# JvanKatwijk/sdr-j-fm

Measured on AMD Instinct MI355X. Metric: IQ MSamples/s demodulated to 48 kHz stereo, higher is better.
Workload: dtype f32 (stage A: 3-term split-f16 MFMA with a per-tile block exponent, f32 accumulate); 1 GPU; config4; population=established, channels_per_gpu=4096, channels_total=4096, streams_per_gpu=4096, block_samples_per_channel=230400, parallelism=channels sharded, 1 rank/GPU

## Files before the change

### sdr-j-fm_amd/csrc/fmx_audio.hip

```cpp
#include "fmx_internal.h"
#include "fmx_fftconv.h"
#include <cstdlib>

namespace fmx {

typedef float v2f __attribute__((ext_vector_type(2)));

__global__ __launch_bounds__(64) void pcm_tail_kernel(DeviceBuffers B, CallGeom G, int channels) {
    const int ch = blockIdx.x * 64 + threadIdx.x + G.ch0;
    if (ch >= G.ch0 + channels) return;
    ChanState *st = &B.state[ch];
    const int frames = (int)(G.M1 - G.M0);
    const int cnt0 = st->pk_cnt;
    float L = st->pk_l, R = st->pk_r;
    int ev = st->pk_events;
    const int tiles = B.peaks_on ? (frames + C_TILE - 1) / C_TILE : 0;
    for (int tile = 0; tile < tiles; tile++) {
        const int i0 = tile * C_TILE, nfr = min(C_TILE, frames - i0);
        const float4 p = B.pk_part[(size_t)ch * B.pk_tiles + tile];
        const int w_first = (cnt0 + i0) / PK_WIN;
        const int to_end = (w_first + 1) * PK_WIN - (cnt0 + i0);
        L = fmaxf(L, p.x); R = fmaxf(R, p.y);
        if (to_end <= nfr) {
            B.pk_ring[(size_t)ch * PK_RING + (ev & (PK_RING - 1))] = make_float2(L, R);
            ev++;
            L = p.z; R = p.w;
        }
    }
    st->pk_l = L; st->pk_r = R; st->pk_events = ev; st->pk_cnt = (cnt0 + frames) % PK_WIN;
    if (B.params[ch].test_tone) st->tt_pos = (int)(((int64_t)st->tt_pos + frames) % TT_CYCLE);
}

constexpr int AF_HIST = (C_MAX_TAPS + 3) / 4 - 1;
constexpr int AF_VALID = 7 * C_TILE;
static_assert(AF_HIST + AF_VALID <= fftc::N, "block + history fit one transform");
static_assert(AUDIO_DELAY % 4 == 0, "the four phases of a frame are one aligned group of four ring entries");
#ifndef AF_WAVES_PER_SIMD
#define AF_WAVES_PER_SIMD 3
#endif
template <bool PEAKS>
__global__ __launch_bounds__(fftc::T, AF_WAVES_PER_SIMD) void audio_fft_kernel(DeviceTables T, DeviceBuffers B, CallGeom G, float2 *__restrict__ pcm) {
    __shared__ __attribute__((aligned(16))) float2 X[fftc::LDS_N];
    __shared__ int pkt[7][4];
    const int ch = blockIdx.y + G.ch0, t = threadIdx.x, lane = t & 63;
    const int64_t mb = G.M0 + (int64_t)blockIdx.x * AF_VALID;
    if (mb >= G.M1) return;
    const ChanParams P = B.params[ch];
    const AudioSet AS = T.audio_sets[P.audio_set];
    const float2 *__restrict__ dring = B.dring + (size_t)ch * (G.dring_mask + 1);
    const float2 *__restrict__ Gs = T.audio_spec + (size_t)P.audio_set * 4 * fftc::N;
    if (PEAKS && t < 28) pkt[t >> 2][t & 3] = 0;
    float2 acc[8];
#pragma unroll
    for (int q = 0; q < 8; q++) acc[q] = make_float2(0.f, 0.f);
    auto load_phase = [&](int p, float2 *a) {
#pragma unroll
        for (int k = 0; k < 8; k++) {
            const int64_t fr = mb - AF_HIST + t + fftc::T * k;
            const int64_t f0 = 4 * fr - AS.delay;
            a[k] = (f0 >= 0 && fr < G.M1) ? dring[(f0 + 3 - p) & G.dring_mask] : make_float2(0.f, 0.f);
        }
    };
    float2 a[8];
    load_phase(0, a);
#pragma unroll 1
    for (int p = 0; p < 4; p++) {
        __syncthreads();
        fftc::forward_slots(t, a, X, T.fft_w);
        fftc::times_spectrum(t, a, Gs + (size_t)p * fftc::N);
#pragma unroll
        for (int q = 0; q < 8; q++) { acc[q].x += a[q].x; acc[q].y += a[q].y; }
        if (p < 3) load_phase(p + 1, a);
    }
    __syncthreads();
    fftc::backward_slots(t, acc, X, T.fft_w);
    const float gl = P.volume * P.left_ch, gr = P.volume * P.right_ch;
    const ChanState *__restrict__ st = &B.state[ch];
    const int64_t F = st->fade_start_frame;
    const int Max = 24000;
    const int cnt0 = st->pk_cnt, tt0 = st->tt_pos;
#pragma unroll
    for (int k = 0; k < 8; k++) {
        const int rel = t + fftc::T * k - AF_HIST;
        const int64_t m = mb + rel;
        const bool live = rel >= 0 && rel < AF_VALID && m < G.M1;
        const int tile = rel >= 0 ? rel / C_TILE : 0;
        float al = acc[k].x * gl, ar = acc[k].y * gr;
        float pv[4] = {0.f, 0.f, 0.f, 0.f};
        if (live) {
            if (G.gain_fix && m - G.M0 < GAIN_FIX_FRAMES) {
                const float2 c = B.gfix[(size_t)ch * GAIN_FIX_FRAMES + (m - G.M0)];
                al += c.x; ar += c.y;
            }
            const int64_t since = m - F;
            if (since >= 0 && since < Max) {
                const float cnt = (float)(Max - (int)since);
                const float f = ((float)Max - cnt) / (float)Max;
                al *= f; ar *= f;
            }
            const int i = (int)(m - G.M0);
            if (P.test_tone) {
#pragma clang fp contract(off)
                const float level = 0.9f;
                al = al * (1.0f - level); ar = ar * (1.0f - level);
                const int pos = (int)(((int64_t)tt0 + i) % TT_CYCLE);
                if (pos >= TT_SILENT) {
                    const float smpl = level * B.tone[pos - TT_SILENT];
                    al = al + smpl; ar = ar + smpl;
                }
            }
            const int i_tile = (int)(mb - G.M0) + tile * C_TILE;
            const bool second = (cnt0 + i) / PK_WIN != (cnt0 + i_tile) / PK_WIN;
            if (PEAKS) { pv[second ? 2 : 0] = fabsf(al); pv[second ? 3 : 1] = fabsf(ar); }
            pcm[(size_t)ch * G.pcm_stride + (m - G.M0)] = make_float2(al, ar);
        }
        if (!PEAKS) {
        } else if (t < 192) {
#pragma unroll
            for (int q = 0; q < 4; q++) {
                int v = __float_as_int(pv[q]);
#define AF_MAX_STEP(ctrl, rmask) v = max(v, __builtin_amdgcn_update_dpp(0, v, ctrl, rmask, 0xf, false))
                AF_MAX_STEP(0x111, 0xf); AF_MAX_STEP(0x112, 0xf); AF_MAX_STEP(0x114, 0xf); AF_MAX_STEP(0x118, 0xf);
                AF_MAX_STEP(0x142, 0xa); AF_MAX_STEP(0x143, 0xc);
#undef AF_MAX_STEP
                if (lane == 63 && k >= 1) atomicMax(&pkt[k - 1][q], v);
            }
        } else if (live) {
#pragma unroll
            for (int q = 0; q < 4; q++) atomicMax(&pkt[tile][q], __float_as_int(pv[q]));
        }
    }
    if (!PEAKS) return;
    __syncthreads();
    const int tiles = (int)(((G.M1 - mb) < AF_VALID ? (G.M1 - mb) : AF_VALID) + C_TILE - 1) / C_TILE;
    if (t < tiles) B.pk_part[(size_t)ch * B.pk_tiles + 7 * blockIdx.x + t] = make_float4(__int_as_float(pkt[t][0]), __int_as_float(pkt[t][1]), __int_as_float(pkt[t][2]), __int_as_float(pkt[t][3]));
}


__global__ __launch_bounds__(GAIN_FIX_BACK) void gain_fix_kernel(DeviceTables T, DeviceBuffers B, CallGeom G, int channels) {
    __shared__ float2 A[GAIN_FIX_BACK];
    const int ch = blockIdx.x, t = threadIdx.x;
    const ChanParams &P = B.params[ch];
    ChanState *st = &B.state[ch];
    const float gl = P.volume * P.left_ch, gr = P.volume * P.right_ch;
    const bool valid = st->gain_valid != 0;
    const float dl = valid ? st->prev_gl - gl : 0.f, dr = valid ? st->prev_gr - gr : 0.f;
    float2 *out = B.gfix + (size_t)ch * GAIN_FIX_FRAMES;
    __syncthreads();
    if (t == 0) { st->prev_gl = gl; st->prev_gr = gr; st->gain_valid = 1; }
    if (dl == 0.f && dr == 0.f) { if (t < GAIN_FIX_FRAMES) out[t] = make_float2(0.f, 0.f); return; }
    const AudioSet AS = T.audio_sets[P.audio_set];
    const float2 *__restrict__ dring = B.dring + (size_t)ch * (G.dring_mask + 1);
    {
        const int q = t;
        float2 acc = make_float2(0.f, 0.f);
        if (q >= 1) {
            const int64_t j = G.J0 - q - AS.delay;
            if (AS.delay > 0) {
                const float *__restrict__ ha = T.audio_lp_taps + (size_t)P.audio_set * AUDIO_TAPS;
                for (int i = 0; i < AUDIO_TAPS; i++) {
                    const int64_t idx = j - i;
                    const float2 v = idx >= 0 ? dring[idx & G.dring_mask] : make_float2(0.f, 0.f);
                    acc.x = fmaf(ha[i], v.x, acc.x); acc.y = fmaf(ha[i], v.y, acc.y);
                }
            } else acc = j >= 0 ? dring[j & G.dring_mask] : make_float2(0.f, 0.f);
        }
        A[q] = acc;
    }
    __syncthreads();
    if (t < GAIN_FIX_FRAMES) {
        const int e = (int)(4 * (G.M0 + t) + 3 - G.J0);
        float2 c = make_float2(0.f, 0.f);
        for (int q = (e < -1 ? -e : 1); q < GAIN_FIX_BACK && e + q < RS_TAPS; q++) {
            const float h = T.rs_taps[e + q];
            c.x = fmaf(h, A[q].x, c.x); c.y = fmaf(h, A[q].y, c.y);
        }
        out[t] = make_float2(dl * c.x, dr * c.y);
    }
}

void launch_gain_fix(const DeviceTables &T, const DeviceBuffers &B, const CallGeom &G, int channels, hipStream_t s) {
    hipLaunchKernelGGL(gain_fix_kernel, dim3(channels), dim3(GAIN_FIX_BACK), 0, s, T, B, G, channels);
}

void launch_audio(const DeviceTables &T, const DeviceBuffers &B, const CallGeom &G, float2 *pcm,
                  int channels, hipStream_t s) {
    const int64_t frames = G.M1 - G.M0;
    if (frames <= 0) return;
    if (B.peaks_on) hipLaunchKernelGGL(audio_fft_kernel<true>, dim3((unsigned)((frames + AF_VALID - 1) / AF_VALID), channels), dim3(fftc::T), 0, s, T, B, G, pcm);
    else hipLaunchKernelGGL(audio_fft_kernel<false>, dim3((unsigned)((frames + AF_VALID - 1) / AF_VALID), channels), dim3(fftc::T), 0, s, T, B, G, pcm);
    hipLaunchKernelGGL(pcm_tail_kernel, dim3((channels + 63) / 64), dim3(64), 0, s, B, G, channels);
}

__global__ __launch_bounds__(256) void conv2_kernel(const float2 *__restrict__ x48, int64_t x_stride, const float *__restrict__ taps,
                                                    int p, int q, int nt, int64_t in0, int64_t out0, int64_t nout,
                                                    float2 *__restrict__ pcm, int64_t pcm_stride) {
    const int64_t i = (int64_t)blockIdx.x * 256 + threadIdx.x;
    if (i >= nout) return;
    const int ch = blockIdx.y;
    const int64_t mq = (out0 + i) * q, n0 = mq / p;
    const int ph = (int)(mq - n0 * p);
    const float *t = taps + (size_t)ph * nt;
    const float2 *x = x48 + (size_t)ch * x_stride + nt + (n0 - in0);
    float ar = 0.f, ai = 0.f;
    for (int k = 0; k < nt; k++) {
        if (n0 - k < 0) break;
        const float2 v = x[-k];
        ar = __fadd_rn(ar, __fmul_rn(t[k], v.x)); ai = __fadd_rn(ai, __fmul_rn(t[k], v.y));
    }
    pcm[(size_t)ch * pcm_stride + i] = make_float2(ar, ai);
}
__global__ __launch_bounds__(256) void conv2_shift_kernel(float2 *x48, int64_t x_stride, int nt, int64_t frames) {
    float2 *x = x48 + (size_t)blockIdx.x * x_stride;
    const int t = threadIdx.x;
    float2 v = make_float2(0.f, 0.f);
    if (t < nt) v = x[frames + t];
    __syncthreads();
    if (t < nt) x[t] = v;
}
void launch_conv2(float2 *x48, int64_t x_stride, const float *taps, int p, int q, int nt, int64_t in0, int64_t frames_in,
                  int64_t out0, int64_t nout, float2 *pcm, int64_t pcm_stride, int channels, hipStream_t s) {
    if (nout > 0)
        hipLaunchKernelGGL(conv2_kernel, dim3((unsigned)((nout + 255) / 256), channels), dim3(256), 0, s, x48, x_stride, taps, p, q, nt,
                           in0, out0, nout, pcm, pcm_stride);
    if (frames_in > 0) hipLaunchKernelGGL(conv2_shift_kernel, dim3(channels), dim3(256), 0, s, x48, x_stride, nt, frames_in);
}

}
```

Baseline: 286,600 MS/s.

## Load ring phase pairs as float4 and hoist FFT twiddles into registers

The audio FFT kernel now reads two polyphase ring entries per float4 load instead of one float2 per phase. When the whole window is in range it takes a fast path with no per-element bounds checks. The FFT twiddles for all three radix-8 stages are loaded once per block and kept in registers for the four forward passes and the backward pass. The spectrum coefficients are prefetched inside the forward FFT so their latency overlaps the LDS stages. The cost is higher register pressure (twiddles plus the float4 buffer), which could lower occupancy at the 3-waves-per-SIMD bound.

```diff
diff --git a/sdr-j-fm_amd/csrc/fmx_audio.hip b/sdr-j-fm_amd/csrc/fmx_audio.hip
--- a/sdr-j-fm_amd/csrc/fmx_audio.hip
+++ b/sdr-j-fm_amd/csrc/fmx_audio.hip
@@ -38,42 +38,110 @@
 #ifndef AF_WAVES_PER_SIMD
 #define AF_WAVES_PER_SIMD 3
 #endif
+__device__ __forceinline__ int af_tid() { int t = threadIdx.x; asm volatile("" : "+v"(t)); return t; }
+struct AfTwiddles { float2 w2048[7], w256[7], w32[7]; };
+__device__ __forceinline__ void af_forward(int t, float2 *a, float2 *X, const AfTwiddles &tw, float4 *hs, const float2 *__restrict__ Hs) {
+    using namespace fftc;
+    int base, j;
+    fwd8(a, tw.w2048); store_q<2048>(a, X, 0, t);
+    __syncthreads();
+    geom8<256>(t, base, j);
+    load_p<256>(a, X, base, j); fwd8(a, tw.w256); store_q<256>(a, X, base, j);
+    const float4 *H4 = reinterpret_cast<const float4 *>(Hs + 8 * t);
+#pragma unroll
+    for (int q = 0; q < 4; q++) hs[q] = H4[q];
+    __syncthreads();
+    geom8<32>(t, base, j);
+    load_p<32>(a, X, base, j); fwd8(a, tw.w32);
+#pragma unroll
+    for (int q = 0; q < 8; q++) {
+        float2 v = a[q];
+        v = quad_f1<-1>(j, v, quad_get<0x4E>(v));
+        a[q] = quad_f2(j, v, quad_get<0xB1>(v));
+    }
+}
+__device__ __forceinline__ void af_backward(int t, float2 *a, float2 *X, const AfTwiddles &tw) {
+    using namespace fftc;
+    int base, j;
+    geom8<32>(t, base, j);
+#pragma unroll
+    for (int q = 0; q < 8; q++) {
+        float2 v = a[q];
+        v = quad_b1<-1>(j, v, quad_get<0xB1>(v));
+        a[q] = quad_b2(j, v, quad_get<0x4E>(v));
+    }
+    inv8(a, tw.w32); store_p<32>(a, X, base, j);
+    __syncthreads();
+    geom8<256>(t, base, j);
+    load_q<256>(a, X, base, j); inv8(a, tw.w256); store_p<256>(a, X, base, j);
+    __syncthreads();
+    load_q<2048>(a, X, 0, t); inv8(a, tw.w2048);
+}
 template <bool PEAKS>
 __global__ __launch_bounds__(fftc::T, AF_WAVES_PER_SIMD) void audio_fft_kernel(DeviceTables T, DeviceBuffers B, CallGeom G, float2 *__restrict__ pcm) {
     __shared__ __attribute__((aligned(16))) float2 X[fftc::LDS_N];
     __shared__ int pkt[7][4];
-    const int ch = blockIdx.y + G.ch0, t = threadIdx.x, lane = t & 63;
+    const int ch = blockIdx.y + G.ch0;
     const int64_t mb = G.M0 + (int64_t)blockIdx.x * AF_VALID;
     if (mb >= G.M1) return;
     const ChanParams P = B.params[ch];
     const AudioSet AS = T.audio_sets[P.audio_set];
     const float2 *__restrict__ dring = B.dring + (size_t)ch * (G.dring_mask + 1);
     const float2 *__restrict__ Gs = T.audio_spec + (size_t)P.audio_set * 4 * fftc::N;
-    if (PEAKS && t < 28) pkt[t >> 2][t & 3] = 0;
-    float2 acc[8];
-#pragma unroll
-    for (int q = 0; q < 8; q++) acc[q] = make_float2(0.f, 0.f);
-    auto load_phase = [&](int p, float2 *a) {
+    if (PEAKS && threadIdx.x < 28) pkt[threadIdx.x >> 2][threadIdx.x & 3] = 0;
+    AfTwiddles tw;
+    {
+        const int t = threadIdx.x;
+        int base, j;
+        fftc::load_tw<2048>(tw.w2048, t, T.fft_w);
+        fftc::geom8<256>(t, base, j); fftc::load_tw<256>(tw.w256, j, T.fft_w);
+        fftc::geom8<32>(t, base, j); fftc::load_tw<32>(tw.w32, j, T.fft_w);
+    }
+    const int64_t f_lo = 4 * (mb - AF_HIST) - AS.delay;
+    const int r_lo = (int)(f_lo & G.dring_mask);
+    const bool plain = f_lo >= 0 && mb - AF_HIST + fftc::N <= G.M1 && r_lo + 4 * (fftc::N - 1) + 3 <= G.dring_mask;
+    auto load_pair = [&](int pp, float4 *b) {
+        const int t = af_tid();
+        if (plain) {
+            const float4 *__restrict__ d = reinterpret_cast<const float4 *>(dring + (r_lo + 4 * t + 2 - 2 * pp));
+#pragma unroll
+            for (int k = 0; k < 8; k++) b[k] = d[2 * fftc::T * k];
+            return;
+        }
 #pragma unroll
         for (int k = 0; k < 8; k++) {
             const int64_t fr = mb - AF_HIST + t + fftc::T * k;
             const int64_t f0 = 4 * fr - AS.delay;
-            a[k] = (f0 >= 0 && fr < G.M1) ? dring[(f0 + 3 - p) & G.dring_mask] : make_float2(0.f, 0.f);
+            b[k] = (f0 >= 0 && fr < G.M1) ? *reinterpret_cast<const float4 *>(dring + ((f0 + 2 - 2 * pp) & G.dring_mask))
+                                          : make_float4(0.f, 0.f, 0.f, 0.f);
         }
     };
-    float2 a[8];
-    load_phase(0, a);
+    float2 acc[8], a[8];
+#pragma unroll
+    for (int q = 0; q < 8; q++) acc[q] = make_float2(0.f, 0.f);
+    auto phase = [&](int p) {
+        __syncthreads();
+        float4 hs[4];
+        af_forward(af_tid(), a, X, tw, hs, Gs + (size_t)p * fftc::N);
+#pragma unroll
+        for (int q = 0; q < 4; q++) { a[2 * q] = fftc::cmul(a[2 * q], make_float2(hs[q].x, hs[q].y)); a[2 * q + 1] = fftc::cmul(a[2 * q + 1], make_float2(hs[q].z, hs[q].w)); }
+#pragma unroll
+        for (int q = 0; q < 8; q++) { acc[q].x += a[q].x; acc[q].y += a[q].y; }
+    };
 #pragma unroll 1
-    for (int p = 0; p < 4; p++) {
-        __syncthreads();
-        fftc::forward_slots(t, a, X, T.fft_w);
-        fftc::times_spectrum(t, a, Gs + (size_t)p * fftc::N);
-#pragma unroll
-        for (int q = 0; q < 8; q++) { acc[q].x += a[q].x; acc[q].y += a[q].y; }
-        if (p < 3) load_phase(p + 1, a);
-    }
-    __syncthreads();
-    fftc::backward_slots(t, acc, X, T.fft_w);
+    for (int pp = 0; pp < 2; pp++) {
+        float4 b[8];
+        load_pair(pp, b);
+#pragma unroll
+        for (int k = 0; k < 8; k++) a[k] = make_float2(b[k].z, b[k].w);
+        phase(2 * pp);
+#pragma unroll
+        for (int k = 0; k < 8; k++) a[k] = make_float2(b[k].x, b[k].y);
+        phase(2 * pp + 1);
+    }
+    __syncthreads();
+    af_backward(af_tid(), acc, X, tw);
+    const int t = af_tid(), lane = t & 63;
     const float gl = P.volume * P.left_ch, gr = P.volume * P.right_ch;
     const ChanState *__restrict__ st = &B.state[ch];
     const int64_t F = st->fade_start_frame;
```

Result: slower. 283,200 MS/s (-1.2%).
